# jean-pierreBoth/kmerutils

Measured on AMD Instinct MI355X. Metric: Gbases/sec k-mer+sketch throughput, k=31, 200 sketches/read, higher is better.
Workload: dtype u64; 1 GPU; ont_k31: 746333 ONT-shaped reads (log-normal lengths, 8% errors), 4.38e+09 bases, k=31, ProbMinHash3a m=200 + kmercount 8-bit; workload_name=ont_k31, reads_per_gpu=746333, bases_per_gpu=4379626696, kmers_per_gpu=4357236706, k=31, sketch_size=200, sketch=True, count=True, parallelism=reads sharded x1

## Files before the change

### kmerutils_amd/csrc/kmu_pmh_points.hip

```cpp
#include "kmu_pmh_steps.h"

namespace kmu {

static constexpr uint32_t PTS_REFRESH_MASK = 15u;

template <bool UNIT_W = false>
__device__ __forceinline__ bool pmh3a_first_point_may_matter(const SketchArgs &a, bool sig32, uint64_t qb, uint64_t key,
                                                             uint32_t w, const double *winv_lut, uint64_t &s0, uint64_t &s3) {
    const uint64_t seed = hasher_finish(KMU_HASHER_NOHASH, key, sig32);
    s0 = splitmix_at(seed, 1);
    s3 = splitmix_at(seed, 4);
    const uint64_t r1 = rotl64(s0 + s3, 23) + s0;
    const double u1 = __longlong_as_double((long long) ((r1 >> 12) | 0x3FF0000000000000ull)) - 1.0;
    const double x = a.e01.c1 * u1;
    if (UNIT_W) return !(x < 1.0) || x < __longlong_as_double((long long) qb);
    return !(x < 1.0) || winv_of(winv_lut, w) * x < __longlong_as_double((long long) qb);
}

__device__ __forceinline__ void pmh3a_first_point_rest(const SketchArgs &a, bool sig32, uint64_t *hmin, uint64_t *sig,
                                                       const uint64_t *qmax_sh, bool have, uint64_t key, uint32_t w,
                                                       uint64_t s0, uint64_t s3, const double *winv_lut) {
    const uint64_t qb = __hip_atomic_load(qmax_sh, __ATOMIC_RELAXED, __HIP_MEMORY_SCOPE_WORKGROUP);
    if (have) {
        const double winv = winv_of(winv_lut, w);
        const uint64_t r1 = rotl64(s0 + s3, 23) + s0;
        const double u1 = __longlong_as_double((long long) ((r1 >> 12) | 0x3FF0000000000000ull)) - 1.0;
        double x = a.e01.c1 * u1;
        const double qmax = __longlong_as_double((long long) qb);
        const bool slow = !(x < 1.0);
        if (slow || winv * x < qmax) {
            const uint64_t seed = hasher_finish(KMU_HASHER_NOHASH, key, sig32);
            Xoshiro rng;
            rng.s0 = s0;
            rng.s3 = s3;
            rng.s1 = splitmix_at(seed, 2);
            rng.s2 = splitmix_at(seed, 3);
            (void) rng.next();
            if (slow) x = exp01_rest(a.e01, rng);
            const double h = winv * x;
            if (h < qmax) slot_update_wave(hmin, sig, draw_slot(a, rng), h, key);
        }
    }
}

__global__ void __launch_bounds__(256) k_pts_long_list(const uint32_t *lst_n, uint32_t n_seq, uint32_t thr, uint32_t *out) {
    const uint32_t r = blockIdx.x * blockDim.x + threadIdx.x;
    if (r < n_seq && lst_n[r] > thr) out[2 + atomicAdd(&out[0], 1u)] = r;
}
__device__ __forceinline__ uint64_t wg4_qmax(const uint64_t *arrays, size_t wave_words, int m) {
    uint64_t q = 0;
    for (int t = lane_id(); t < m; t += 64) {
        uint64_t v = H_INIT;
#pragma unroll
        for (int w4 = 0; w4 < 4; w4++) {
            const uint64_t x = __hip_atomic_load(&arrays[(size_t) w4 * wave_words + t], __ATOMIC_RELAXED, __HIP_MEMORY_SCOPE_WORKGROUP);
            v = x < v ? x : v;
        }
        q = v > q ? v : q;
    }
    return wave_max_u64(q);
}

template <bool SIG32, bool WG>
__device__ __forceinline__ void pts_one_read(const SketchArgs &a, uint32_t r, uint8_t *smem, size_t wave_words, const double *winv_lut) {
    const int wave = threadIdx.x >> 6, lane = lane_id();
    constexpr bool sig32 = SIG32;
    constexpr uint32_t cstride = WG ? 256u : 64u;
    const uint32_t cstart = WG ? 64u * (uint32_t) wave : 0u;
    uint64_t *arrays = reinterpret_cast<uint64_t *>(smem);
    uint64_t *hmin = arrays + (size_t) wave * wave_words;
    uint64_t *sig = hmin + a.m;
    uint64_t *qmax_sh = sig + a.m;
    uint64_t *qk = qmax_sh + 2;
    uint32_t *qw = reinterpret_cast<uint32_t *>(qk + 128);
    uint64_t *qs0 = qk + 128 + 64, *qs3 = qs0 + 128;
    const uint64_t base = a.offsets[r] - a.offsets[0];
    const uint32_t n = uniform_u32(a.lst_n[r]);
    const uint32_t n_u = uniform_u32(a.lst_nu[r]);
    uint64_t tau_b = H_INIT;
    if (n >= a.tau_min_n) {
        const uint64_t len = a.offsets[r + 1] - a.offsets[r];
        const uint64_t kk = (uint64_t) a.cfg.k;
        const double tau = a.tau_num / (double) (len >= kk ? len - kk + 1 : 0);
        if (tau < 1.0) tau_b = (uint64_t) __double_as_longlong(tau);
        tau_b = uniform_u64(tau_b);
    }
    uint32_t wmax = 0;
    uint64_t qb = H_INIT;
    for (int turn = 0; turn < 2; turn++) {
        for (int t = lane; t < a.m; t += 64) { hmin[t] = H_INIT; sig[t] = 0; }
        if (lane == 0) *qmax_sh = tau_b;
        if (WG) __syncthreads();
        uint32_t chunk = 0, qn = 0;
        qb = tau_b;
        uint64_t key_nx = 0;
        uint32_t w_nx = 1;
        {
            const uint32_t i = cstart + (uint32_t) lane;
            if (i < n) { key_nx = a.lst_keys[base + i]; w_nx = i < n_u ? 1u : a.lst_w[base + i]; }
        }
        for (uint32_t c = cstart; c < n; c += cstride, chunk++) {
            const uint32_t i = c + (uint32_t) lane;
            const uint64_t key = key_nx;
            const uint32_t w = w_nx;
            const bool have = i < n && w != 0u;
            if (have) wmax = w > wmax ? w : wmax;
            if (i + cstride < n) key_nx = a.lst_keys[base + i + cstride];
            w_nx = 1u;
            if (c + cstride + 64u > n_u) {
                if (i + cstride < n && i + cstride >= n_u) w_nx = a.lst_w[base + i + cstride];
            }
            if ((chunk & (WG && chunk < 64u ? PTS_REFRESH_MASK >> 2 : PTS_REFRESH_MASK)) == 0u) {
                qb = WG ? wg4_qmax(arrays, wave_words, a.m) : wave_qmax(hmin, a.m);
                qb = qb < tau_b ? qb : tau_b;
                if (lane == 0) *qmax_sh = qb;
            }
            uint64_t s0 = 0, s3 = 0;
            const bool pass = c + 64u <= n_u ? have && pmh3a_first_point_may_matter<true>(a, sig32, qb, key, w, winv_lut, s0, s3)
                                             : have && pmh3a_first_point_may_matter(a, sig32, qb, key, w, winv_lut, s0, s3);
            const uint64_t pm = __ballot(pass);
            if (pass) {
                const uint32_t pos = qn + (uint32_t) __popcll(pm & ((1ull << lane) - 1ull));
                qk[pos] = key;
                qw[pos] = w;
                qs0[pos] = s0;
                qs3[pos] = s3;
            }
            qn += (uint32_t) __popcll(pm);
            if (qn >= 64u) {
                qn -= 64u;
                pmh3a_first_point_rest(a, sig32, hmin, sig, qmax_sh, true, qk[qn + lane], qw[qn + lane], qs0[qn + lane], qs3[qn + lane],
                                       winv_lut);
            }
        }
        if (qn) {
            const bool have = (uint32_t) lane < qn;
            pmh3a_first_point_rest(a, sig32, hmin, sig, qmax_sh, have, have ? qk[lane] : 0ull, have ? qw[lane] : 1u, have ? qs0[lane] : 0ull,
                                   have ? qs3[lane] : 0ull, winv_lut);
        }
        if (WG) {
            __syncthreads();
            qb = wg4_qmax(arrays, wave_words, a.m);
        } else qb = wave_qmax(hmin, a.m);
        if (tau_b == H_INIT || qb < tau_b) break;
        tau_b = H_INIT;
        if (lane == 0 && (!WG || wave == 0)) atomicAdd(a.tau_redo, 1u);
        if (WG) __syncthreads();
    }
    wmax = (uint32_t) wave_max_u64((uint64_t) wmax);
    if (n && wmax && winv_of(winv_lut, wmax) < __longlong_as_double((long long) qb)) {
        const uint32_t c0 = 1.0 < __longlong_as_double((long long) qb) ? 0u : (n_u & ~63u);
        uint32_t c = cstart;
        if (c < c0) c += (c0 - c + cstride - 1u) / cstride * cstride;
        for (; c < n; c += cstride) {
            const uint32_t i = c + (uint32_t) lane;
            double winv = 0.0;
            bool alive = false;
            if (i < n) {
                const uint32_t w = i < n_u ? 1u : a.lst_w[base + i];
                winv = winv_of(winv_lut, w);
                alive = w != 0u && winv < __longlong_as_double((long long) qb);
            }
            if (__any(alive)) pmh3a_more_points<true>(a, sig32, hmin, sig, qb, alive, alive ? a.lst_keys[base + i] : 0ull, winv);
        }
    }
    if (WG) {
        __syncthreads();
        for (int t = threadIdx.x; t < a.m; t += 256) {
            uint64_t bh = arrays[t], bk = arrays[a.m + t];
#pragma unroll
            for (int w4 = 1; w4 < 4; w4++) {
                const uint64_t h = arrays[(size_t) w4 * wave_words + t], kk = arrays[(size_t) w4 * wave_words + a.m + t];
                if (h < bh || (h == bh && kk < bk)) { bh = h; bk = kk; }
            }
            const uint64_t v = bh == H_INIT ? 0ull : bk;
            if (sig32) reinterpret_cast<uint32_t *>(a.sig_out)[(uint64_t) r * a.m + t] = (uint32_t) v;
            else reinterpret_cast<uint64_t *>(a.sig_out)[(uint64_t) r * a.m + t] = v;
        }
        __syncthreads();
    } else {
        for (int t = lane; t < a.m; t += 64) {
            const uint64_t v = hmin[t] == H_INIT ? 0ull : sig[t];
            if (sig32) reinterpret_cast<uint32_t *>(a.sig_out)[(uint64_t) r * a.m + t] = (uint32_t) v;
            else reinterpret_cast<uint64_t *>(a.sig_out)[(uint64_t) r * a.m + t] = v;
        }
    }
}

template <bool SIG32>
__global__ void __launch_bounds__(256) k_pmh_points(SketchArgs a) {
    extern __shared__ __attribute__((aligned(16))) uint8_t smem[];
    const int lane = lane_id();
    const size_t wave_words = 2 * (size_t) a.m + PTS_WAVE_WORDS;
    double *winv_lut = reinterpret_cast<double *>(reinterpret_cast<uint64_t *>(smem) + (size_t) 4 * wave_words);
    for (uint32_t t = threadIdx.x; t < WINV_LUT; t += blockDim.x) winv_lut[t] = winv_entry(t);
    __syncthreads();
    uint32_t n_long = a.pts_long ? a.pts_long[0] : 0u;
    if (n_long > 4u * gridDim.x) n_long = 0u;
    for (uint32_t li = blockIdx.x; li < n_long; li += gridDim.x) pts_one_read<SIG32, true>(a, a.pts_long[2 + li], smem, wave_words, winv_lut);
    uint32_t q_next = 0, q_end = 0;
    for (;;) {
        const uint32_t r = wave_take(a.queue2, q_next, q_end, lane);
        if (r >= a.n_seq) break;
        if (n_long && uniform_u32(a.lst_n[r]) > a.pts_long_t) continue;
        pts_one_read<SIG32, false>(a, r, smem, wave_words, winv_lut);
    }
}

__global__ void __launch_bounds__(256) k_pmh_reduce(const uint64_t *part_h, const uint64_t *part_k, uint64_t n_parts, int m,
                                                    uint64_t stride, int sig_bytes, void *sig_out, uint64_t *part_out) {
    __shared__ uint64_t sh[256], sk[256];
    const int t = blockIdx.x;
    uint64_t bh = H_INIT, bk = 0;
    for (uint64_t i = threadIdx.x; i < n_parts; i += blockDim.x) {
        const uint64_t h = part_h[i * stride + t], key = part_k[i * stride + t];
        if (h < bh || (h == bh && h != H_INIT && key < bk)) { bh = h; bk = key; }
    }
    sh[threadIdx.x] = bh;
    sk[threadIdx.x] = bk;
    __syncthreads();
    for (int d = 128; d >= 1; d >>= 1) {
        if ((int) threadIdx.x < d) {
            const uint64_t h = sh[threadIdx.x + d], key = sk[threadIdx.x + d];
            if (h < sh[threadIdx.x] || (h == sh[threadIdx.x] && h != H_INIT && key < sk[threadIdx.x])) {
                sh[threadIdx.x] = h;
                sk[threadIdx.x] = key;
            }
        }
        __syncthreads();
    }
    if (threadIdx.x == 0) {
        if (part_out) {
            part_out[t] = sh[0];
            part_out[m + t] = sk[0];
            return;
        }
        const uint64_t v = sh[0] == H_INIT ? 0ull : sk[0];
        if (sig_bytes == 4) reinterpret_cast<uint32_t *>(sig_out)[t] = (uint32_t) v;
        else reinterpret_cast<uint64_t *>(sig_out)[t] = v;
    }
}

#define KMU_X_INST(...) template __global__ void __VA_ARGS__(SketchArgs);
KMU_PMH_POINTS_FORMS(KMU_X_INST)
#undef KMU_X_INST

}
```

### kmerutils_amd/csrc/kmu_pmh_uq.hip

```cpp
#include "kmu_pmh_steps.h"

namespace kmu {

__device__ __forceinline__ void vm_wait_lds_loads() {
    __builtin_amdgcn_s_waitcnt(0x0F70);
    asm volatile("" ::: "memory");
}

template <int UQ_THREADS, uint32_t UQ_BM_BITS, uint32_t UQ_COLL, int MINW>
__global__ void __launch_bounds__(UQ_THREADS, MINW) k_multiset_uq(SketchArgs a) {
    typedef UqShape<UQ_THREADS, UQ_BM_BITS, UQ_COLL> SH;
    constexpr uint32_t UQ_KEYS = SH::KEYS, UQ_BM_WORDS = SH::BM_WORDS, UQ_BUCKETS = SH::BUCKETS, UQ_TILE = SH::TILE;
    static_assert((UQ_BM_WORDS / 4) % (uint32_t) UQ_THREADS == 0, "whole 16-byte stores per thread wipe a bitmap");
    static_assert(UQ_COLL % UQ_THREADS == 0 && UQ_COLL / UQ_THREADS <= 4, "collected keys per thread");
    static_assert((uint32_t) UQ_THREADS <= UQ_BM_WORDS, "every thread has a word of bitmap A of its own");
    extern __shared__ __attribute__((aligned(16))) uint8_t smem[];
    uint32_t *bmA = reinterpret_cast<uint32_t *>(smem);
    uint32_t *bmB = bmA + UQ_BM_WORDS;
    uint64_t *ck = reinterpret_cast<uint64_t *>(bmB + UQ_BM_WORDS);
    uint64_t *dk = ck + UQ_COLL;
    uint32_t *dw = reinterpret_cast<uint32_t *>(dk + UQ_COLL);
    uint32_t *bst = dw + UQ_COLL;
    uint32_t *words = bst + UQ_BUCKETS + 1;
    uint32_t *wtot = words + UQ_TILE;
    uint32_t *misc = wtot + UQ_THREADS / 64;
    constexpr uint32_t RAW_OFF = ((8u * UQ_BM_WORDS + 20u * UQ_COLL + 4u * (UQ_BUCKETS + 1u + UQ_TILE + (uint32_t) UQ_THREADS / 64u) + 64u) + 15u) & ~15u;
    uint8_t *rawp = smem + RAW_OFF;
    const KmerCfg cfg = a.cfg;
    const int k = cfg.k, tid = threadIdx.x, lane = lane_id(), wave = tid >> 6;
    for (uint32_t i = tid; i < UQ_BUCKETS + 1; i += UQ_THREADS) bst[i] = 0;
    auto take = [&]() -> uint32_t {
        if (misc[8] == misc[9]) {
            if (!misc[11]) misc[10] = atomicAdd(KMU_COLD_ARG(queue), (uint32_t) QCHUNK);
            misc[8] = misc[10];
            misc[9] = misc[10] + QCHUNK;
            misc[11] = 0;
        }
        const uint32_t v = misc[8]++;
        if (misc[8] == misc[9] && !misc[11]) { misc[10] = atomicAdd(KMU_COLD_ARG(queue), (uint32_t) QCHUNK); misc[11] = 1; }
        return v;
    };
    if (tid == 0) {
        misc[8] = misc[9] = misc[10] = misc[11] = 0;
        misc[4] = take();
        misc[5] = take();
        misc[6] = take();
    }
    __syncthreads();
    const uint64_t off_first = uniform_u64(a.offsets[0]);
    const uint64_t total = a.total_bytes ? a.total_bytes : uniform_u64(a.offsets[a.n_seq]);
    auto seq_of = [&](uint32_t q) -> uint32_t {
        const uint32_t *rl = KMU_COLD_ARG(read_list);
        return rl ? rl[q] : q;
    };
    uint32_t r = uniform_u32(misc[4]);
    uint32_t rs = r < a.n_queue ? uniform_u32(seq_of(r)) : 0u;
    SeqView sv;
    sv.base = a.bases; sv.packed = 0; sv.total = total; sv.begin = 0; sv.len = 0;
    if (r < a.n_queue) { sv.begin = uniform_u64(a.offsets[rs]); sv.len = uniform_u64(a.offsets[rs + 1]) - sv.begin; }
    auto fits = [&](const SeqView &v) -> bool {
        const uint32_t Lv = v.len >= 0x80000000ull ? 0xFFFFFFFFu : (uint32_t) v.len;
        return Lv >= (uint32_t) k && Lv - (uint32_t) k + 1u + seq_lead(v) <= UQ_KEYS;
    };
    static_assert(UQ_KREG % 4 == 0 && UQ_THREADS % 4 == 0, "quarters of words");
    auto place_of = [&](int q) -> uint32_t { return 4u * ((uint32_t) tid + (uint32_t) UQ_THREADS * (uint32_t) (q >> 2)) + (uint32_t) (q & 3); };
    uint32_t r_next = uniform_u32(misc[5]);
    uint32_t rs_next = r_next < a.n_queue ? uniform_u32(seq_of(r_next)) : 0u;
    SeqView nv = sv;
    bool nv_mine = false;
    if (r_next < a.n_queue) {
        nv.begin = uniform_u64(a.offsets[rs_next]);
        nv.len = uniform_u64(a.offsets[rs_next + 1]) - nv.begin;
        nv_mine = fits(nv);
    }
    uint32_t r_nn = uniform_u32(misc[6]);
    uint32_t rs_nn = r_nn < a.n_queue ? uniform_u32(seq_of(r_nn)) : 0u;
    __syncthreads();
    uint32_t pf_bad = 0;
    bool pf_valid = false;
    auto n_words = [&](const SeqView &v) -> uint32_t {
        const uint32_t Lv = (uint32_t) v.len, ld = seq_lead(v);
        return (uint32_t) ((Lv - 1 + ld) >> 4) + 2;
    };
    while (r < a.n_queue) {
        if (tid == 0) {
            misc[6] = take();
            misc[0] = 0;
            misc[1] = 0;
        }
        const uint32_t L = sv.len >= 0x80000000ull ? 0xFFFFFFFFu : (uint32_t) sv.len;
        const uint32_t nk = L >= (uint32_t) k ? L - (uint32_t) k + 1u : 0u;
        const bool mine = nk >= 1u && nk + seq_lead(sv) <= UQ_KEYS;
        uint32_t bad = 0;
        if (L == 0 && tid == 0) atomicOr(KMU_COLD_ARG(err), DERR_EMPTY_SEQ);
        if (nk == 0) bad |= wave_validate_seq(sv, wave, UQ_THREADS / 64, false);
        const uint32_t lead = seq_lead(sv), wfirst = lead >> 4;
        if (mine) {
            const uint32_t nw = n_words(sv);
            if (pf_valid) bad |= pf_bad;
            else {
                for (uint32_t t = tid; t < nw; t += UQ_THREADS) {
                    uint32_t b;
                    words[t] = load_code_word(sv, (uint64_t) wfirst + t, b);
                    bad |= b;
                }
            }
            uint4 *za = reinterpret_cast<uint4 *>(bmA), *zb = reinterpret_cast<uint4 *>(bmB);
#pragma unroll
            for (uint32_t z = 0; z < UQ_BM_WORDS / 4 / (uint32_t) UQ_THREADS; z++) {
                za[tid + z * UQ_THREADS] = make_uint4(0u, 0u, 0u, 0u);
                zb[tid + z * UQ_THREADS] = make_uint4(0u, 0u, 0u, 0u);
            }
        }
        lds_barrier();
        const bool has_nn = r_nn < a.n_queue;
        const uint32_t r_n3 = uniform_u32(misc[6]);
        const uint32_t rs_n3 = r_n3 < a.n_queue ? seq_of(r_n3) : 0u;
        const uint64_t nn_o0 = has_nn ? a.offsets[rs_nn] : 0ull, nn_o1 = has_nn ? a.offsets[rs_nn + 1] : 0ull;
        uint32_t nwn = 0, wfn = 0;
        if (nv_mine) {
            nwn = n_words(nv);
            wfn = seq_lead(nv) >> 4;
#pragma unroll
            for (int u = 0; u < 3; u++) {
                const uint32_t tw = (uint32_t) tid + (uint32_t) u * UQ_THREADS;
                if (tw < nwn && chunk_is_plain(nv, (uint64_t) wfn + tw))
                    chunk16_to_lds_uncounted(nv.base + (nv.begin & ~15ull) + 16 * ((uint64_t) wfn + tw),
                                             lds_addr(smem) + RAW_OFF + (uint32_t) (wave + u * (UQ_THREADS / 64)) * 1024u);
            }
        }
        uint64_t rk[UQ_KREG];
        auto bm_index = [&](uint64_t key) -> uint32_t {
            return (((uint32_t) key ^ (uint32_t) (key >> 32)) * 0x85EBCA6Bu) >> (32 - UQ_BM_BITS);
        };
        const uint32_t span = uniform_u32(nk + (lead - 16u * wfirst));
        auto group_used = [&](int q0) -> bool { return 4u * (uint32_t) UQ_THREADS * (uint32_t) (q0 >> 2) < span; };
        bool over = false;
        if (mine) {
            const uint32_t l0 = lead - 16u * wfirst;
            auto key_phase = [&](auto fast_tag) __attribute__((always_inline)) {
                constexpr bool FAST = decltype(fast_tag)::value;
                const int kq = (int) opaque_u32((uint32_t) k);
#pragma unroll
                for (int q0 = 0; q0 < UQ_KREG; q0 += 4) {
                    if (!group_used(q0)) {
#pragma unroll
                        for (int u = 0; u < 4; u++) rk[q0 + u] = __builtin_nondeterministic_value(rk[q0 + u]);
                        continue;
                    }
                    uint32_t bit[4], rbw[4], rbb[4];
                    const uint32_t wi = ((uint32_t) tid >> 2) + (uint32_t) (UQ_THREADS / 4) * (uint32_t) (q0 >> 2);
                    const StepWin sw = step_win(words[wi], words[wi + 1], words[wi + 2], kq);
#pragma unroll
                    for (int u = 0; u < 4; u++) {
                        const int q = q0 + u;
                        rbw[u] = (uint32_t) tid;
                        rbb[u] = 0;
                        rk[q] = 0;
                        if (place_of(q) - l0 < nk) {
                            uint64_t val, rc;
                            step_val_rc_lane(sw, 4u * ((uint32_t) tid & 3u) + (uint32_t) u, val, rc);
                            const uint64_t key = FAST ? int64_hash(rc < val ? rc : val) : apply_fhash(cfg, val, rc);
                            rk[q] = key;
                            const uint32_t bi = bm_index(key);
                            rbw[u] = bi >> 5;
                            rbb[u] = 1u << (bi & 31u);
                        }
                    }
#pragma unroll
                    for (int u = 0; u < 4; u++) bit[u] = atomicOr(&bmA[rbw[u]], rbb[u]);
#pragma unroll
                    for (int u = 0; u < 4; u++) bit[u] &= rbb[u];
#pragma unroll
                    for (int u = 0; u < 4; u++)
                        if (bit[u]) atomicOr(&bmB[rbw[u]], bit[u]);
                }
            };
            if (cfg.fhash == KMU_FHASH_CANON_INVHASH && cfg.kmer_type == KMU_KMER64BIT) key_phase(std::true_type{});
            else key_phase(std::false_type{});
            lds_barrier();
        }
        if (nv_mine) {
            vm_wait_lds_loads();
            pf_bad = 0;
#pragma unroll
            for (int u = 0; u < 3; u++) {
                const uint32_t tw = (uint32_t) tid + (uint32_t) u * UQ_THREADS;
                uint32_t b = 0;
                if (tw < nwn)
                    words[tw] = chunk_is_plain(nv, (uint64_t) wfn + tw)
                                    ? code_word_from_chunk(nv, (uint64_t) wfn + tw, *reinterpret_cast<const u32x4 *>(rawp + (size_t) tw * 16), b)
                                    : load_code_word(nv, (uint64_t) wfn + tw, b);
                pf_bad |= b;
            }
        }
        const uint64_t lb = sv.begin - off_first;
        if (mine) {
#pragma unroll
            for (int q0 = 0; q0 < UQ_KREG; q0 += 4) {
                if (!group_used(q0)) continue;
                bool uq[4], co[4];
                uint64_t um[4], cm[4];
                uint32_t ut = 0, ct = 0, bw[4];
#pragma unroll
                for (int u = 0; u < 4; u++) bw[u] = bmB[bm_index(rk[q0 + u]) >> 5];
#pragma unroll
                for (int u = 0; u < 4; u++) {
                    const int q = q0 + u;
                    const bool have = place_of(q) - (lead - 16u * wfirst) < nk;
                    co[u] = have && (bw[u] & (1u << (bm_index(rk[q]) & 31u))) != 0u;
                    uq[u] = have && !co[u];
                }
#pragma unroll
                for (int u = 0; u < 4; u++) {
                    um[u] = __ballot(uq[u]);
                    cm[u] = __ballot(co[u]);
                    ut += (uint32_t) __popcll(um[u]);
                    ct += (uint32_t) __popcll(cm[u]);
                }
                uint32_t ub = 0, cb = 0;
                const uint32_t ln = opaque_lane_u32((uint32_t) lane), z0 = opaque_lane_u32(0u);
                if (ln == 0) {
                    if (ut) ub = atomicAdd(lane_ptr(misc, z0), ut);
                    if (ct) cb = atomicAdd(lane_ptr(misc + 1, z0), ct);
                }
                ub = bcast_u32(ub, 0);
                cb = bcast_u32(cb, 0);
#pragma unroll
                for (int u = 0; u < 4; u++) {
                    const uint64_t below = (1ull << lane) - 1ull;
                    if (uq[u]) {
                        const uint64_t at = lb + ub + (uint32_t) __popcll(um[u] & below);
                        a.lst_keys[at] = rk[q0 + u];
                    }
                    if (co[u]) {
                        const uint32_t at = cb + (uint32_t) __popcll(cm[u] & below);
                        if (at < UQ_COLL) ck[at] = rk[q0 + u];
                    }
                    ub += (uint32_t) __popcll(um[u]);
                    cb += (uint32_t) __popcll(cm[u]);
                }
            }
            lds_barrier();
            const uint32_t n_u = uniform_u32(misc[0]), n_c = uniform_u32(misc[1]);
            over = n_c > UQ_COLL;
            if (!over && n_c) {
                uint64_t key[UQ_COLL / UQ_THREADS];
                uint32_t rb[UQ_COLL / UQ_THREADS];
#pragma unroll
                for (int j = 0; j < (int) (UQ_COLL / UQ_THREADS); j++) {
                    const uint32_t i = (uint32_t) j * UQ_THREADS + tid;
                    rb[j] = 0xFFFFFFFFu;
                    key[j] = 0;
                    if (i < n_c) {
                        key[j] = ck[i];
                        const uint32_t b = mix32(key[j]) / (0x80000000u / (UQ_BUCKETS / 2));
                        rb[j] = (b << 16) | atomicAdd(&bst[b], 1u);
                    }
                }
                lds_barrier();
                {
                    const uint32_t c0 = bst[2 * tid], c1 = bst[2 * tid + 1];
                    const uint32_t incl = wave_incl_scan_u32(c0 + c1);
                    if (lane == 63) wtot[wave] = incl;
                    lds_barrier();
                    uint32_t pre = incl - (c0 + c1);
#pragma unroll
                    for (int w = 0; w < UQ_THREADS / 64; w++) pre += w < wave ? wtot[w] : 0u;
                    bst[2 * tid] = pre;
                    bst[2 * tid + 1] = pre + c0;
                }
                lds_barrier();
#pragma unroll
                for (int j = 0; j < (int) (UQ_COLL / UQ_THREADS); j++)
                    if (rb[j] != 0xFFFFFFFFu) {
                        const uint32_t pos = bst[rb[j] >> 16] + (rb[j] & 0xFFFFu);
                        rb[j] = (rb[j] & 0xFFFF0000u) | pos;
                        dk[pos] = key[j];
                        dw[pos] = 1u;
                    }
                lds_barrier();
#pragma unroll
                for (int j = 0; j < (int) (UQ_COLL / UQ_THREADS); j++)
                    if (rb[j] != 0xFFFFFFFFu) {
                        const uint32_t pos = rb[j] & 0xFFFFu;
                        for (uint32_t t = bst[rb[j] >> 16]; t < pos; t++)
                            if (dk[t] == key[j]) {
                                dw[pos] = 0u;
                                atomicAdd(&dw[t], 1u);
// ... 46 lines not shown
```

### kmerutils_amd/csrc/kmu_sketch_kernels.h

```cpp
#pragma once

#include "kmu_ctx.hpp"
#include "kmu_device.h"

namespace kmu {

struct SketchArgs {
    const uint8_t *bases;
    const uint64_t *offsets;
    const uint64_t *packed_offsets;
    const uint64_t *block_rows;
    uint32_t n_seq;
    int packed;
    uint64_t total_bytes;
    KmerCfg cfg;
    int m;
    int hasher;
    int rand08;
    int sig_bytes;
    uint32_t block_size;
    uint32_t cap;
    uint32_t part_target;
    double inv_part_target;
    uint32_t tile_shift;
    uint64_t *scr_keys;
    uint32_t *scr_info;
    uint32_t *scr_w;
    uint32_t skip_longer;
    uint64_t *def_keys;
    int bk_shift;
    uint32_t bk_mask;
    uint32_t *tau_redo;
    double tau_num;
    uint32_t *counts_out;
    const void *hashed;
    int hashed_bytes;
    uint64_t *part_h;
    uint64_t *part_k;
    uint64_t *lst_keys;
    uint32_t *lst_w;
    uint32_t *lst_n;
    uint32_t *lst_nu;
    uint32_t *queue2;
    uint32_t *pts_long;
    uint32_t pts_long_t;
    uint32_t *redo_list;
    const uint32_t *read_list;
    uint32_t n_queue;
    uint32_t tile_words;
    uint32_t idx_thresh;
    uint64_t idx_zone;
    uint32_t tau_min_n;
    Exp01 e01;
    void *sig_out;
    uint32_t *queue;
    uint32_t *err;
};
#define KMU_COLD_ARG(f) kernarg_at<decltype(SketchArgs::f)>((uint32_t) offsetof(SketchArgs, f))

enum { M_READ = 0, M_NSCR = 1, M_NEXT = 2, M_DEF = 3, M_QMAX = 4 , M_FLAGS = 6 , M_WORDS = 8 };
static constexpr uint32_t DEF_CAP = 1u << 20;
static constexpr uint32_t DEF_PARTS = 32;
static constexpr uint32_t DEF_SEG = DEF_CAP / DEF_PARTS;
static constexpr uint32_t LONG_SEQ_KMERS = 1u << 18;
static constexpr int BUCKET_BITS = 12;
static constexpr uint32_t NBUCKETS = 1u << BUCKET_BITS;
static constexpr int QCHUNK = 4;
static constexpr int KREG = 10;
static constexpr uint32_t WINV_LUT = 256;
static constexpr size_t PTS_WAVE_WORDS = 2 + 128 + 64 + 256;
static constexpr double PTS_TAU_C = 4.6;
static constexpr int UQ_KREG = 20;
static constexpr uint32_t UQ1_BM = 17, UQ1_COLL = 1024, UQ2_BM = 18, UQ2_COLL = 2048;
template <int UQ_THREADS, uint32_t UQ_BM_BITS, uint32_t UQ_COLL>
struct UqShape {
    static constexpr uint32_t KEYS = (uint32_t) UQ_THREADS * UQ_KREG;
    static constexpr uint32_t BM_WORDS = (1u << UQ_BM_BITS) / 32;
    static constexpr uint32_t BUCKETS = 2u * UQ_THREADS;
    static constexpr uint32_t TILE = (KEYS + 32 + 15) / 16 + 3;
    static constexpr uint32_t RAW_WAVES = (TILE + 63) / 64;
    static constexpr size_t LDS = (size_t) BM_WORDS * 8 + (size_t) UQ_COLL * 20 + ((size_t) BUCKETS + 1 + TILE + UQ_THREADS / 64 + 8 + 8) * 4 + 64 +
                                  (size_t) RAW_WAVES * 1024 + 16;
};
static constexpr uint32_t SHORT_KEYS = 256, SHORT_SLOTS = 512, SHORT_WORDS = 24;
static constexpr size_t SHORT_WAVE_BYTES = (size_t) SHORT_SLOTS * 12 + SHORT_WORDS * 4;
static constexpr uint32_t SMALLK_WORDS = 32768;
static constexpr uint32_t SMALLK_TILE = 1024;

template <bool AA, bool BOTTOMK, bool EMIT = false, bool PLAIN = false>
__global__ void __launch_bounds__(1024) k_sketch_pmh3a(SketchArgs a);
__global__ void k_pts_long_list(const uint32_t *lst_n, uint32_t n_seq, uint32_t thr, uint32_t *out);
template <bool SIG32>
__global__ void __launch_bounds__(256) k_pmh_points(SketchArgs a);
template <int UQ_THREADS, uint32_t UQ_BM_BITS, uint32_t UQ_COLL, int MINW>
__global__ void __launch_bounds__(UQ_THREADS, MINW) k_multiset_uq(SketchArgs a);
__global__ void __launch_bounds__(1024, 4) k_multiset_long(SketchArgs a);
__global__ void k_multiset_short(SketchArgs a);
template <bool SIG32>
__global__ void __launch_bounds__(256) k_pmh_points_short(SketchArgs a);
template <bool EMIT>
__global__ void __launch_bounds__(1024) k_sketch_smallk(SketchArgs a);
__global__ void k_pmh_reduce(const uint64_t *part_h, const uint64_t *part_k, uint64_t n_parts, int m, uint64_t stride, int sig_bytes, void *sig_out,
                             uint64_t *part_out);
__global__ void k_max_len(const uint64_t *offsets, uint32_t n_seq, uint64_t *out);
__global__ void k_nk_scan(const uint64_t *offsets, uint32_t n_seq, int k, uint64_t *koff, uint32_t *err);
__global__ void k_seq_hashes_compact(const uint8_t *bases, const uint64_t *offsets, const uint64_t *packed_offsets, uint32_t n_seq, int packed,
                                     uint64_t total, KmerCfg cfg, const uint64_t *koff, uint64_t *out, uint32_t *err, int spread);
__global__ void k_widen_u32(const uint32_t *in, uint64_t n, uint64_t *out);

#define KMU_PMH_GENERAL_FORMS(X)                                                                                                    \
    X(k_sketch_pmh3a<false, false>) X(k_sketch_pmh3a<false, false, true>) X(k_sketch_pmh3a<true, true>) X(k_sketch_pmh3a<true, false>) \
    X(k_sketch_pmh3a<false, true>) X(k_sketch_pmh3a<false, false, false, true>)
#define KMU_PMH_POINTS_FORMS(X) X(k_pmh_points<true>) X(k_pmh_points<false>)
#define KMU_PMH_SHORT_FORMS(X) X(k_pmh_points_short<true>) X(k_pmh_points_short<false>)
#define KMU_PMH_UQ_FORMS(X) X(k_multiset_uq<512, UQ1_BM, UQ1_COLL, 4>) X(k_multiset_uq<1024, UQ2_BM, UQ2_COLL, 4>)
#define KMU_PMH_SMALLK_FORMS(X) X(k_sketch_smallk<true>) X(k_sketch_smallk<false>)
#define KMU_SKETCH_KERNEL_FORMS(X) \
    KMU_PMH_GENERAL_FORMS(X) KMU_PMH_POINTS_FORMS(X) KMU_PMH_SHORT_FORMS(X) KMU_PMH_UQ_FORMS(X) KMU_PMH_SMALLK_FORMS(X)
#define KMU_X_EXTERN(...) extern template __global__ void __VA_ARGS__(SketchArgs);
KMU_SKETCH_KERNEL_FORMS(KMU_X_EXTERN)
#undef KMU_X_EXTERN

}
```

### kmerutils_amd/csrc/kmu_sketch_pmh.hip

```cpp
#include <algorithm>
#include <cmath>

#include "kmu_sketch_host.hpp"
#include "kmu_sketch_kernels.h"

using namespace kmu;

static int atoi_or(const char *s, int dflt) { return s ? atoi(s) : dflt; }

static bool smallk_route(const kmu_sketch_params *p, int hashed_bytes, bool partial, bool blocks) {
    if (p->algo != KMU_ALGO_PROB3A || p->kmer_type != KMU_KMER32BIT || p->kmer_size > 8 || hashed_bytes || partial || blocks ||
        p->block_size != 0 || p->sketch_size > 512)
        return false;
    switch (p->fhash) {
    case KMU_FHASH_IDENTITY_RAW: case KMU_FHASH_VALUE_MASKED: case KMU_FHASH_CANON_RAW: case KMU_FHASH_CANON_INVHASH:
    case KMU_FHASH_INVHASH_RAW: case KMU_FHASH_CANON_VALUE: break;
    default: return false;
    }
    return atoi_or(getenv("KMU_PMH_SMALLK"), 1) != 0;
}

enum class PmhRoute { SMALLK, SHORT, UQ, LISTS, ONE_PASS, GENERAL };
struct PmhPlan {
    PmhRoute route = PmhRoute::GENERAL;
    bool lists = false;
    uint64_t list_bases = 0;
    uint32_t pts_long = 32768;
    int cus = 0;
};

static int alloc_lists(kmu_ctx *ctx, SketchArgs &a, uint64_t bases) {
    void *ln;
    KMU_TRY(dev_array(ctx, "cnt.partA", bases + 8, &a.lst_keys));
    KMU_TRY(dev_array(ctx, "pmh.lst_w", bases + 16, &a.lst_w));
    KMU_TRY(dev_buf(ctx, "pmh.lst_n", (size_t) a.n_seq * 8 + 64, &ln));
    a.lst_n = (uint32_t *) ln;
    a.lst_nu = a.lst_n + a.n_seq;
    KMU_HIP(ctx, hipMemsetAsync(a.lst_nu, 0, (size_t) a.n_seq * 4, ctx->stream));
    return KMU_OK;
}

static int pmh_route(kmu_ctx *ctx, const kmu_sketch_params *p, const DevSeqs &ds, const PmhInputs &in, PmhPlan *plan) {
    const int split_mode = atoi_or(getenv("KMU_PMH_SPLIT"), -1);
    const bool plain_on = atoi_or(getenv("KMU_PMH_PLAIN"), 1) != 0;
    const bool short_on = atoi_or(getenv("KMU_PMH_SHORT"), 1) != 0;
    plan->pts_long = (uint32_t) std::max(0, atoi_or(getenv("KMU_PMH_PTS_LONG"), 32768));
    const int cus = ctx->num_cus;
    plan->cus = std::max(cus / 2, cus - std::max(0, atoi_or(getenv("KMU_PMH_RESERVE_CUS"), 0)));
    const bool smallk = smallk_route(p, in.hashed_bytes, in.part_h != nullptr, in.d_block_rows != nullptr);
    const bool whole = p->algo != KMU_ALGO_BOTTOMK && !kmer_is_aa(p->kmer_type) && !in.hashed_bytes && !in.part_h &&
                       !in.d_block_rows && p->block_size == 0;
    bool lists = (size_t) 4 * (2 * (size_t) p->sketch_size + PTS_WAVE_WORDS) * 8 + WINV_LUT * 8 <= 150 * 1024 &&
                 split_mode != 0 && (smallk || (whole && !in.skip_longer && (split_mode == 1 || in.len_stats)));
    const bool judge = !smallk && split_mode != 1;
    if (lists) {
        uint64_t &total = plan->list_bases;
        if (in.len_stats) total = in.len_stats[1];
        else if (!ds.h_offsets.empty()) total = ds.h_offsets[ds.n_seq] - ds.h_offsets[0];
        else {
            uint64_t ends[2] = {0, 0};
            KMU_HIP(ctx, hipMemcpyAsync(&ends[0], ds.offsets, 8, hipMemcpyDeviceToHost, ctx->stream));
            KMU_HIP(ctx, hipMemcpyAsync(&ends[1], ds.offsets + ds.n_seq, 8, hipMemcpyDeviceToHost, ctx->stream));
            KMU_HIP(ctx, hipStreamSynchronize(ctx->stream));
            total = ends[1] - ends[0];
        }
        if (judge) {
            const uint64_t longest = in.len_stats[0];
            const double cu_share = (double) ctx->num_cus / 256.0;
            const double wave_rate = plan->pts_long && longest > plan->pts_long ? 1.6e5 : 4.0e4;
            const double t_ideal = (double) total / (2.35e8 * cu_share), t_tail = (double) longest / wave_rate;
            const double overhang = t_tail >= t_ideal ? t_tail - 0.5 * t_ideal : t_tail * t_tail / (2.0 * t_ideal);
            const double gain = 0.43 * (double) total / (4.9e7 * cu_share);
            if (gain <= overhang + 0.02) lists = false;
        }
        if (lists && (smallk || judge)) {
            const size_t need_k = total * 8 + 64, need_w = total * 4 + 64;
            size_t grow = 0, free_b = 0, total_b = 0;
            if (ctx->bufs["cnt.partA"].bytes < need_k) grow += need_k + need_k / 8;
            if (ctx->bufs["pmh.lst_w"].bytes < need_w) grow += need_w + need_w / 8;
            if (grow && hipMemGetInfo(&free_b, &total_b) == hipSuccess && free_b < grow + total_b / 8) lists = false;
        }
    }
    plan->lists = lists;
    const bool plain = whole && !ds.packed && plain_on;
    const bool short_reads = in.len_stats && in.len_stats[0] < (uint64_t) SHORT_KEYS + (uint64_t) p->kmer_size && short_on;
    plan->route = smallk         ? PmhRoute::SMALLK
                  : lists && plain ? (short_reads ? PmhRoute::SHORT : PmhRoute::UQ)
                  : lists          ? PmhRoute::LISTS
                  : plain          ? PmhRoute::ONE_PASS
                                   : PmhRoute::GENERAL;
    return KMU_OK;
}

static int alloc_queue(kmu_ctx *ctx, SketchArgs &a) {
    void *q;
    KMU_TRY(dev_buf(ctx, "queue", 256, &q));
    KMU_HIP(ctx, hipMemsetAsync(q, 0, 256, ctx->stream));
    a.queue = (uint32_t *) q;
    return KMU_OK;
}

static int launch_points(kmu_ctx *ctx, SketchArgs a, int cus, uint32_t thr) {
    void (*const kpts)(SketchArgs) = a.sig_bytes == 4 ? k_pmh_points<true> : k_pmh_points<false>;
    const size_t lds2 = (size_t) 4 * (2 * (size_t) a.m + PTS_WAVE_WORDS) * 8 + WINV_LUT * 8;
    if (lds2 > 64 * 1024)
        KMU_HIP(ctx, hipFuncSetAttribute((const void *) kpts, hipFuncAttributeMaxDynamicSharedMemorySize, 160 * 1024));
    const int per_cu = (int) std::max<size_t>(1, std::min<size_t>(8, (160 * 1024) / lds2));
    const int grid2 = (int) std::max<uint64_t>(1, std::min<uint64_t>(((uint64_t) a.n_seq + 3) / 4, (uint64_t) cus * per_cu));
    a.pts_long = nullptr;
    a.pts_long_t = thr;
    if (thr && a.n_seq) {
        if (thr < 1024u) a.pts_long_t = thr = 1024u;
        KMU_TRY(dev_array(ctx, "pts.long", (size_t) a.n_seq + 2 + 16, &a.pts_long));
        KMU_HIP(ctx, hipMemsetAsync(a.pts_long, 0, 8, ctx->stream));
        KMU_TRY(launch(ctx, nullptr, k_pts_long_list, dim3((a.n_seq + 255) / 256), dim3(256), 0, a.lst_n, a.n_seq, thr, a.pts_long));
    }
    if (!ctx->pmh_tau_read) {
        const char *e = getenv("KMU_PMH_TAU_C");
        ctx->pmh_tau_c = !e ? PTS_TAU_C : (!strcmp(e, "off") ? 0.0 : atof(e));
        ctx->pmh_tau_read = true;
    }
    const bool fresh = !ctx->bufs.count("pmh.tau_redo");
    void *tr;
    KMU_TRY(dev_buf(ctx, "pmh.tau_redo", 4, &tr));
    if (fresh) KMU_HIP(ctx, hipMemsetAsync(tr, 0, 4, ctx->stream));
    a.tau_redo = (uint32_t *) tr;
    a.tau_num = (double) a.m * (std::log((double) a.m) + ctx->pmh_tau_c);
    a.tau_min_n = ctx->pmh_tau_c != 0.0 && a.tau_num > 0.0 ? (uint32_t) std::min(a.tau_num, 4.0e9) : 0xFFFFFFFFu;
    return launch(ctx, "k_pmh_points", kpts, dim3(grid2), dim3(256), lds2, a);
}

typedef void (*sketch_kernel_t)(SketchArgs);

static int launch_main(kmu_ctx *ctx, const SketchArgs &a, sketch_kernel_t kern, int grid, size_t lds, const char *name) {
    return launch(ctx, name, kern, dim3(grid), dim3(1024), lds, a);
}

static int launch_smallk(kmu_ctx *ctx, SketchArgs a, const PmhPlan &plan) {
    const sketch_kernel_t kern = plan.lists ? k_sketch_smallk<true> : k_sketch_smallk<false>;
    const size_t lds_fixed = (size_t) SMALLK_WORDS * 4 + (plan.lists ? 0 : (size_t) 16 * a.m) + ((size_t) SMALLK_TILE + 2) * 4 + 64;
    a.cap = (uint32_t) ((160 * 1024 - lds_fixed) / 2) & ~2047u;
    if (a.cap > 32768u) a.cap = 32768u;
    const size_t lds = lds_fixed + (size_t) a.cap * 2;
    KMU_HIP(ctx, hipFuncSetAttribute((const void *) kern, hipFuncAttributeMaxDynamicSharedMemorySize, 160 * 1024));
    KMU_TRY(alloc_queue(ctx, a));
    a.queue2 = a.queue + 48;
    const int grid = (int) std::max<uint64_t>(1, std::min<uint64_t>((uint64_t) a.n_seq, (uint64_t) plan.cus));
    KMU_TRY(launch_main(ctx, a, kern, grid, lds, "k_sketch_smallk"));
    if (plan.lists) KMU_TRY(launch_points(ctx, a, plan.cus, plan.pts_long));
    return KMU_OK;
}

struct PmhShape {
    size_t lds;
    uint64_t slots;
    int grid;
};

static int pmh_shape(kmu_ctx *ctx, const kmu_sketch_params *p, SketchArgs &a, sketch_kernel_t kern, bool plain, int cus, PmhShape *g) {
    const bool bottomk = p->algo == KMU_ALGO_BOTTOMK, aa = kmer_is_aa(p->kmer_type) || a.hashed_bytes != 0;
    a.bk_shift = (a.sig_bytes == 4 && p->hasher == KMU_HASHER_NOHASH) ? 20 : 52;
    a.bk_mask = p->hasher == KMU_HASHER_INT64HASH ? 0xFFu : 0xFFFFu;
    hipFuncAttributes fa;
    KMU_HIP(ctx, hipFuncGetAttributes(&fa, (const void *) kern));
    size_t lds_max = 160 * 1024 - fa.sharedSizeBytes;
    if (hipFuncSetAttribute((const void *) kern, hipFuncAttributeMaxDynamicSharedMemorySize, (int) lds_max) != hipSuccess) {
        (void) hipGetLastError();
        lds_max = 64 * 1024;
    }
    const sketch_kernel_t kern_redo = k_sketch_pmh3a<false, false>;
    if (plain && lds_max > 64 * 1024 &&
        hipFuncSetAttribute((const void *) kern_redo, hipFuncAttributeMaxDynamicSharedMemorySize, (int) lds_max) != hipSuccess)
        return fail(ctx, KMU_E_HIP, "hipFuncSetAttribute failed for the general sketch kernel");
    a.tile_words = (aa && !bottomk) ? 4 : (lds_max > 64 * 1024 || bottomk ? 4096 + 2 : 1024 + 2);
    size_t fixed = (size_t) 16 * a.m + 4 * ((size_t) NBUCKETS + 1 + 8) + 4 * (M_WORDS + 16 + DEF_PARTS) +
                   4 * ((size_t) a.tile_words + 4) + 64;
    if (fixed + 12 * 256 > lds_max) return fail(ctx, KMU_E_UNSUPPORTED, "sketch_size %d too large for LDS", a.m);
    uint32_t cap = (uint32_t) ((lds_max - fixed) / 12);
    cap &= ~63u;
    if (cap > 65472) cap = 65472;
    a.cap = cap;
    a.part_target = cap - cap / 10;
    a.inv_part_target = 1.0 / (double) a.part_target;
    if (plain && a.part_target > (uint32_t) KREG * 1024u)
        return fail(ctx, KMU_E_HIP, "internal: a single pass (%u k-mers) must fit the register keys of the PLAIN kernel", a.part_target);
    const uint32_t tp = (a.tile_words - 2) * 16;
    a.tile_shift = 0;
    while ((1u << a.tile_shift) < tp) a.tile_shift++;
    if ((1u << a.tile_shift) != tp) return fail(ctx, KMU_E_HIP, "internal: tile size %u is not a power of two", tp);
    g->lds = (size_t) 12 * cap + fixed;
    KMU_TRY(alloc_queue(ctx, a));
    g->slots = (uint64_t) cus * std::max<int>(1, (int) (lds_max / g->lds));
    g->grid = (int) std::max<uint64_t>(1, std::min<uint64_t>((uint64_t) a.n_seq, g->slots));
    KMU_TRY(dev_array(ctx, "pmh.scr_keys", (size_t) g->grid * cap, &a.scr_keys));
    KMU_TRY(dev_array(ctx, "pmh.scr_info", (size_t) g->grid * cap, &a.scr_info));
    KMU_TRY(dev_array(ctx, "pmh.scr_w", (size_t) g->grid * cap, &a.scr_w));
    KMU_TRY(dev_array(ctx, "pmh.def_keys", (size_t) g->grid * DEF_CAP, &a.def_keys));
    if (plain) KMU_TRY(dev_array(ctx, "pmh.redo", (size_t) a.n_seq + 16, &a.redo_list));
    return KMU_OK;
}

static int launch_listed(kmu_ctx *ctx, SketchArgs a, sketch_kernel_t kern, const PmhShape &g, uint32_t n, const char *name) {
    KMU_HIP(ctx, hipMemsetAsync(a.queue, 0, 256, ctx->stream));
    a.read_list = a.redo_list;
    a.n_queue = n;
    return launch_main(ctx, a, kern, (int) std::min<uint64_t>((uint64_t) n, g.slots), g.lds, name);
}

static int read_count(kmu_ctx *ctx, const SketchArgs &a, uint32_t *n) {
    KMU_HIP(ctx, hipMemcpyAsync(n, a.queue + 56, 4, hipMemcpyDeviceToHost, ctx->stream));
    KMU_HIP(ctx, hipStreamSynchronize(ctx->stream));
    return KMU_OK;
}

static int launch_short(kmu_ctx *ctx, const SketchArgs &a, int cus) {
    const size_t lds_s = 4 * SHORT_WAVE_BYTES;
    const int per_cu = 5;
    KMU_TRY(launch(ctx, "k_multiset_short", k_multiset_short,
                   dim3((unsigned) std::max<uint64_t>(1, std::min<uint64_t>(((uint64_t) a.n_seq + 3) / 4, (uint64_t) cus * per_cu))), dim3(256),
                   lds_s, a));
    KMU_HIP(ctx, hipMemsetAsync(a.queue, 0, 256, ctx->stream));
    const sketch_kernel_t kpts = a.sig_bytes == 4 ? k_pmh_points_short<true> : k_pmh_points_short<false>;
    const size_t lds2 = (size_t) 4 * (2 * (size_t) a.m + 2) * 8 + WINV_LUT * 8;
    if (lds2 > 64 * 1024)
        KMU_HIP(ctx, hipFuncSetAttribute((const void *) kpts, hipFuncAttributeMaxDynamicSharedMemorySize, 160 * 1024));
    const int per_cu2 = (int) std::max<size_t>(1, std::min<size_t>(4, (160 * 1024) / lds2));
    const int grid2 = (int) std::max<uint64_t>(1, std::min<uint64_t>(((uint64_t) a.n_seq + 3) / 4, (uint64_t) cus * per_cu2));
    return launch(ctx, "k_pmh_points_short", kpts, dim3(grid2), dim3(256), lds2, a);
}

static int launch_uq(kmu_ctx *ctx, SketchArgs a, sketch_kernel_t kern, const PmhShape &g, const PmhPlan &plan) {
    {
        const auto ka = k_multiset_uq<512, UQ1_BM, UQ1_COLL, 4>;
        const size_t lds_a = UqShape<512, UQ1_BM, UQ1_COLL>::LDS;
        KMU_HIP(ctx, hipFuncSetAttribute((const void *) ka, hipFuncAttributeMaxDynamicSharedMemorySize, 80 * 1024));
        KMU_TRY(launch(ctx, "k_multiset_uq", ka, dim3((unsigned) std::max<uint64_t>(1, std::min<uint64_t>(a.n_seq, (uint64_t) plan.cus * 2))),
                       dim3(512), lds_a, a));
    }
    uint32_t n_long = 0;
    KMU_TRY(read_count(ctx, a, &n_long));
    if (n_long) {
        const auto kb = k_multiset_uq<1024, UQ2_BM, UQ2_COLL, 4>;
        const size_t lds_b = UqShape<1024, UQ2_BM, UQ2_COLL>::LDS;
        uint32_t *rl2;
        KMU_TRY(dev_array(ctx, "pmh.redo2", (size_t) a.n_seq + 16, &rl2));
        KMU_HIP(ctx, hipFuncSetAttribute((const void *) kb, hipFuncAttributeMaxDynamicSharedMemorySize, 160 * 1024));
        KMU_HIP(ctx, hipMemsetAsync(a.queue, 0, 256, ctx->stream));
        SketchArgs b = a;
        b.read_list = a.redo_list;
        b.redo_list = rl2;
        b.n_queue = n_long;
        KMU_TRY(launch(ctx, "k_multiset_uq", kb, dim3((unsigned) std::max<uint64_t>(1, std::min<uint64_t>(n_long, (uint64_t) plan.cus))), dim3(1024),
                       lds_b, b));
        KMU_TRY(read_count(ctx, a, &n_long));
        if (n_long) {
            KMU_HIP(ctx, hipFuncSetAttribute((const void *) k_multiset_long, hipFuncAttributeMaxDynamicSharedMemorySize, 160 * 1024));
            KMU_HIP(ctx, hipMemsetAsync(a.queue, 0, 256, ctx->stream));
            SketchArgs c = a;
            c.read_list = rl2;
            c.n_queue = n_long;
            const uint64_t grid_c = std::min<uint64_t>(std::min<uint64_t>(n_long, (uint64_t) plan.cus), (uint64_t) g.grid);
            KMU_TRY(launch(ctx, "k_sketch_pmh3a", k_multiset_long, dim3((unsigned) std::max<uint64_t>(1, grid_c)), dim3(1024), lds_b, c));
            KMU_TRY(read_count(ctx, a, &n_long));
        }
    }
    if (n_long) KMU_TRY(launch_listed(ctx, a, kern, g, n_long, "k_sketch_pmh3a"));
    KMU_HIP(ctx, hipMemsetAsync(a.queue, 0, 256, ctx->stream));
    return launch_points(ctx, a, plan.cus, plan.pts_long);
}

static int launch_one_pass(kmu_ctx *ctx, const SketchArgs &a, sketch_kernel_t kern, const PmhShape &g) {
    KMU_TRY(launch_main(ctx, a, kern, g.grid, g.lds, "k_sketch_pmh3a"));
    uint32_t n_redo = 0;
    KMU_TRY(read_count(ctx, a, &n_redo));
    if (n_redo) KMU_TRY(launch_listed(ctx, a, k_sketch_pmh3a<false, false>, g, n_redo, "k_sketch_pmh3a_redo"));
    return KMU_OK;
}

static SketchArgs sketch_args(const kmu_sketch_params *p, const DevSeqs &ds, void *d_sig, uint32_t *d_err, const PmhInputs &in) {
    SketchArgs a;
    memset(&a, 0, sizeof a);
// ... 131 lines not shown
```

Measured before the change: 53.93 Gbases/s.

## Split points loop into unit-weight and weighted phases and defer qmax refresh

Splits the k_pmh_points main loop into a unit-weight phase, specialised at compile time to skip weight loads, winv lookups and qw stores, and a separate weighted tail phase. It also holds off the periodic qmax reduction for the first half of the chunks when a tau bound is active, so the threshold comes only from tau early in the read. It also changes the UQ kernel's group_used check to account for the per-wave offset, which skips unused groups. The risks are weaker early filtering when qmax reduction is delayed and correctness subtleties in the qw fixup between the two phases.

```diff
diff --git a/kmerutils_amd/csrc/kmu_pmh_points.hip b/kmerutils_amd/csrc/kmu_pmh_points.hip
--- a/kmerutils_amd/csrc/kmu_pmh_points.hip
+++ b/kmerutils_amd/csrc/kmu_pmh_points.hip
@@ -17,18 +17,19 @@
     return !(x < 1.0) || winv_of(winv_lut, w) * x < __longlong_as_double((long long) qb);
 }
 
+template <bool UNIT_W = false>
 __device__ __forceinline__ void pmh3a_first_point_rest(const SketchArgs &a, bool sig32, uint64_t *hmin, uint64_t *sig,
                                                        const uint64_t *qmax_sh, bool have, uint64_t key, uint32_t w,
                                                        uint64_t s0, uint64_t s3, const double *winv_lut) {
     const uint64_t qb = __hip_atomic_load(qmax_sh, __ATOMIC_RELAXED, __HIP_MEMORY_SCOPE_WORKGROUP);
     if (have) {
-        const double winv = winv_of(winv_lut, w);
+        const double winv = UNIT_W ? 1.0 : winv_of(winv_lut, w);
         const uint64_t r1 = rotl64(s0 + s3, 23) + s0;
         const double u1 = __longlong_as_double((long long) ((r1 >> 12) | 0x3FF0000000000000ull)) - 1.0;
         double x = a.e01.c1 * u1;
         const double qmax = __longlong_as_double((long long) qb);
         const bool slow = !(x < 1.0);
-        if (slow || winv * x < qmax) {
+        if (slow || (UNIT_W ? x : winv * x) < qmax) {
             const uint64_t seed = hasher_finish(KMU_HASHER_NOHASH, key, sig32);
             Xoshiro rng;
             rng.s0 = s0;
@@ -37,7 +38,7 @@
             rng.s2 = splitmix_at(seed, 3);
             (void) rng.next();
             if (slow) x = exp01_rest(a.e01, rng);
-            const double h = winv * x;
+            const double h = UNIT_W ? x : winv * x;
             if (h < qmax) slot_update_wave(hmin, sig, draw_slot(a, rng), h, key);
         }
     }
@@ -85,7 +86,7 @@
         if (tau < 1.0) tau_b = (uint64_t) __double_as_longlong(tau);
         tau_b = uniform_u64(tau_b);
     }
-    uint32_t wmax = 0;
+    uint32_t wmax = n_u ? 1u : 0u;
     uint64_t qb = H_INIT;
     for (int turn = 0; turn < 2; turn++) {
         for (int t = lane; t < a.m; t += 64) { hmin[t] = H_INIT; sig[t] = 0; }
@@ -93,46 +94,51 @@
         if (WG) __syncthreads();
         uint32_t chunk = 0, qn = 0;
         qb = tau_b;
+        const uint32_t hold = tau_b != H_INIT && n > cstart ? (uint32_t) (((uint64_t) ((n - cstart + cstride - 1u) / cstride) * a.tau_hold) >> 8) : 0u;
         uint64_t key_nx = 0;
         uint32_t w_nx = 1;
         {
             const uint32_t i = cstart + (uint32_t) lane;
             if (i < n) { key_nx = a.lst_keys[base + i]; w_nx = i < n_u ? 1u : a.lst_w[base + i]; }
         }
-        for (uint32_t c = cstart; c < n; c += cstride, chunk++) {
+        uint32_t c = cstart;
+        auto step = [&](auto unit_tag) __attribute__((always_inline)) {
+            constexpr bool UNIT = decltype(unit_tag)::value;
             const uint32_t i = c + (uint32_t) lane;
             const uint64_t key = key_nx;
-            const uint32_t w = w_nx;
-            const bool have = i < n && w != 0u;
-            if (have) wmax = w > wmax ? w : wmax;
+            const uint32_t w = UNIT ? 1u : w_nx;
+            const bool have = UNIT || (i < n && w != 0u);
+            if (!UNIT && have) wmax = w > wmax ? w : wmax;
             if (i + cstride < n) key_nx = a.lst_keys[base + i + cstride];
-            w_nx = 1u;
+            if (!UNIT) w_nx = 1u;
             if (c + cstride + 64u > n_u) {
                 if (i + cstride < n && i + cstride >= n_u) w_nx = a.lst_w[base + i + cstride];
             }
-            if ((chunk & (WG && chunk < 64u ? PTS_REFRESH_MASK >> 2 : PTS_REFRESH_MASK)) == 0u) {
+            if ((chunk & (WG && chunk < 64u ? PTS_REFRESH_MASK >> 2 : PTS_REFRESH_MASK)) == 0u && chunk >= hold) {
                 qb = WG ? wg4_qmax(arrays, wave_words, a.m) : wave_qmax(hmin, a.m);
                 qb = qb < tau_b ? qb : tau_b;
                 if (lane == 0) *qmax_sh = qb;
             }
             uint64_t s0 = 0, s3 = 0;
-            const bool pass = c + 64u <= n_u ? have && pmh3a_first_point_may_matter<true>(a, sig32, qb, key, w, winv_lut, s0, s3)
-                                             : have && pmh3a_first_point_may_matter(a, sig32, qb, key, w, winv_lut, s0, s3);
+            const bool pass = have && pmh3a_first_point_may_matter<UNIT>(a, sig32, qb, key, w, winv_lut, s0, s3);
             const uint64_t pm = __ballot(pass);
             if (pass) {
                 const uint32_t pos = qn + (uint32_t) __popcll(pm & ((1ull << lane) - 1ull));
                 qk[pos] = key;
-                qw[pos] = w;
+                if (!UNIT) qw[pos] = w;
                 qs0[pos] = s0;
                 qs3[pos] = s3;
             }
             qn += (uint32_t) __popcll(pm);
             if (qn >= 64u) {
                 qn -= 64u;
-                pmh3a_first_point_rest(a, sig32, hmin, sig, qmax_sh, true, qk[qn + lane], qw[qn + lane], qs0[qn + lane], qs3[qn + lane],
-                                       winv_lut);
-            }
-        }
+                pmh3a_first_point_rest<UNIT>(a, sig32, hmin, sig, qmax_sh, true, qk[qn + lane], UNIT ? 1u : qw[qn + lane], qs0[qn + lane],
+                                             qs3[qn + lane], winv_lut);
+            }
+        };
+        for (; c + 64u <= n_u; c += cstride, chunk++) step(std::true_type{});
+        if ((uint32_t) lane < qn) qw[lane] = 1u;
+        for (; c < n; c += cstride, chunk++) step(std::false_type{});
         if (qn) {
             const bool have = (uint32_t) lane < qn;
             pmh3a_first_point_rest(a, sig32, hmin, sig, qmax_sh, have, have ? qk[lane] : 0ull, have ? qw[lane] : 1u, have ? qs0[lane] : 0ull,
diff --git a/kmerutils_amd/csrc/kmu_pmh_uq.hip b/kmerutils_amd/csrc/kmu_pmh_uq.hip
--- a/kmerutils_amd/csrc/kmu_pmh_uq.hip
+++ b/kmerutils_amd/csrc/kmu_pmh_uq.hip
@@ -134,7 +134,8 @@
             return (((uint32_t) key ^ (uint32_t) (key >> 32)) * 0x85EBCA6Bu) >> (32 - UQ_BM_BITS);
         };
         const uint32_t span = uniform_u32(nk + (lead - 16u * wfirst));
-        auto group_used = [&](int q0) -> bool { return 4u * (uint32_t) UQ_THREADS * (uint32_t) (q0 >> 2) < span; };
+        const uint32_t wave_first = 256u * uniform_u32((uint32_t) tid >> 6);
+        auto group_used = [&](int q0) -> bool { return 4u * (uint32_t) UQ_THREADS * (uint32_t) (q0 >> 2) + wave_first < span; };
         bool over = false;
         if (mine) {
             const uint32_t l0 = lead - 16u * wfirst;
diff --git a/kmerutils_amd/csrc/kmu_sketch_kernels.h b/kmerutils_amd/csrc/kmu_sketch_kernels.h
--- a/kmerutils_amd/csrc/kmu_sketch_kernels.h
+++ b/kmerutils_amd/csrc/kmu_sketch_kernels.h
@@ -51,6 +51,7 @@
     uint32_t idx_thresh;
     uint64_t idx_zone;
     uint32_t tau_min_n;
+    uint32_t tau_hold;
     Exp01 e01;
     void *sig_out;
     uint32_t *queue;
@@ -70,6 +71,7 @@
 static constexpr uint32_t WINV_LUT = 256;
 static constexpr size_t PTS_WAVE_WORDS = 2 + 128 + 64 + 256;
 static constexpr double PTS_TAU_C = 4.6;
+static constexpr uint32_t PTS_TAU_HOLD = 128;
 static constexpr int UQ_KREG = 20;
 static constexpr uint32_t UQ1_BM = 17, UQ1_COLL = 1024, UQ2_BM = 18, UQ2_COLL = 2048;
 template <int UQ_THREADS, uint32_t UQ_BM_BITS, uint32_t UQ_COLL>
diff --git a/kmerutils_amd/csrc/kmu_sketch_pmh.hip b/kmerutils_amd/csrc/kmu_sketch_pmh.hip
--- a/kmerutils_amd/csrc/kmu_sketch_pmh.hip
+++ b/kmerutils_amd/csrc/kmu_sketch_pmh.hip
@@ -127,6 +127,7 @@
     a.tau_redo = (uint32_t *) tr;
     a.tau_num = (double) a.m * (std::log((double) a.m) + ctx->pmh_tau_c);
     a.tau_min_n = ctx->pmh_tau_c != 0.0 && a.tau_num > 0.0 ? (uint32_t) std::min(a.tau_num, 4.0e9) : 0xFFFFFFFFu;
+    a.tau_hold = PTS_TAU_HOLD;
     return launch(ctx, "k_pmh_points", kpts, dim3(grid2), dim3(256), lds2, a);
 }
 
```

Result: faster. 54.91 Gbases/s, median of 6 (+1.8%).
